# PotatoSpudowski/fastLLaMa

Hardware: NVIDIA H100
Metric: tokens/sec LLaMA-7B q4_0 decode (n_batch=1, greedy) (higher is better)
Workload: dtype u8

## Files before the change

### fastllama_b200/csrc/fl_token_kernel.cu

```cuda
#include <cuda_fp16.h>
#include <stdlib.h>

#include <algorithm>
#include <vector>

#include "fl_common.cuh"
#include "fl_decode.h"
#include "fl_decode_dev.cuh"
#include "fl_exact.cuh"
#include "fl_kernels.h"

#define TK_CW 16
#define TK_NT (TK_CW * 32)
#define TK_TG 4
#define TK_WPG 4
#define TK_GMAX 4
#define TK_CHB 32
#define TK_PW 4
#define TK_THREADS (TK_NT + 32 * TK_PW)
#define TK_REGS_CONSUMER 104
#define TK_REGS_PRODUCER 64

enum { TK_PH_MATVEC = 0, TK_PH_ATTN = 1 };

struct tk_phase {
    int kind;
    int nb, nchunks;
    uint32_t srow;
    int swiglu;
    int units[3];
    uint32_t row_bytes;
    fl_mv_args a;
    const float *q, *kcache, *vcache;
    float *out;
    int k_row_stride, n_head, head_dim, n_ctx;
    int head_split;
    int out_ll, out_seq, n_out_peer;
    float *out_peer[7];
    float scale;
};

struct tk_params {
    const tk_phase *phases;
    int n_phases;
    unsigned *grid_bar;
    unsigned *err;
    int rank, world;
    unsigned *ll_count;
    int n_ll;
    const uint16_t *exp_tab;
    unsigned long long *prof;
    unsigned *prof2;
    int S, Sg;
    uint32_t grid_magic, grid_shift, s_magic, s_shift;
    uint32_t slot_bytes;
    int diag;
    uint32_t off_y, off_red, off_rowbuf, off_cnt, off_sc, off_stage0;
};

__device__ __forceinline__ unsigned long long tk_now() {
    unsigned long long t;
    asm volatile("mov.u64 %0, %globaltimer;" : "=l"(t));
    return t;
}
__device__ __forceinline__ void tk_bar_consumers(int id) { asm volatile("bar.sync %0, %1;" ::"r"(id), "r"(TK_NT) : "memory"); }

__device__ __forceinline__ void tk_wait_ge(const unsigned *p, unsigned target, bool sys, unsigned *err, unsigned who) {
    unsigned long long t0 = 0;
    for (unsigned n = 1;; n++) {
        unsigned v;
        if (sys) asm volatile("ld.relaxed.sys.global.u32 %0, [%1];" : "=r"(v) : "l"(p) : "memory");
        else asm volatile("ld.acquire.gpu.global.u32 %0, [%1];" : "=r"(v) : "l"(p) : "memory");
        if ((int)(v - target) >= 0) return;
        if ((n & 1023u) == 0) {
            if (*(volatile unsigned *)err) return;
            const unsigned long long t = tk_now();
            if (t0 == 0) t0 = t;
            else if (t - t0 > 2000000000ull) {
                if (atomicExch(err, 1u) == 0u) { err[1] = who; err[2] = target; err[3] = v; err[4] = blockIdx.x; }
                return;
            }
        }
    }
}
__device__ __forceinline__ void tk_mbar_wait(uint32_t bar, uint32_t parity, unsigned *err, unsigned who, unsigned slot) {
    unsigned long long t0 = 0;
    for (unsigned n = 1; !fl_mbar_try_wait(bar, parity); n++) {
        if ((n & 4095u) == 0) {
            if (*(volatile unsigned *)err) return;
            const unsigned long long t = tk_now();
            if (t0 == 0) t0 = t;
            else if (t - t0 > 2000000000ull) {
                if (atomicExch(err, 1u) == 0u) { err[1] = who; err[2] = slot; err[3] = parity; err[4] = blockIdx.x; }
                return;
            }
        }
    }
}
__device__ __forceinline__ void tk_tag_wait(volatile uint32_t *tag, uint32_t want, unsigned *err, unsigned who, unsigned slot) {
    unsigned long long t0 = 0;
    for (unsigned n = 1; *tag != want; n++) {
        if ((n & 4095u) == 0) {
            if (*(volatile unsigned *)err) return;
            const unsigned long long t = tk_now();
            if (t0 == 0) t0 = t;
            else if (t - t0 > 2000000000ull) {
                if (atomicExch(err, 1u) == 0u) { err[1] = who; err[2] = slot; err[3] = want; err[4] = blockIdx.x; }
                return;
            }
        }
    }
}
__device__ __forceinline__ void tk_grid_sync(const tk_params &prm, unsigned target, unsigned) {
    tk_bar_consumers(13);
    if (threadIdx.x == 0) {
        asm volatile("red.release.gpu.global.add.u32 [%0], 1;" ::"l"(prm.grid_bar) : "memory");
        tk_wait_ge(prm.grid_bar, target, false, prm.err, 0x100u);
    }
    tk_bar_consumers(13);
}

struct tk_slice {
    int f0, f1, f2, n0, n1, n2, t0, t1, ntiles;
};
__device__ __forceinline__ uint32_t tk_div(uint32_t n, uint32_t magic, uint32_t shift) { return (magic ? __umulhi(n, magic) : n) >> shift; }
__device__ __forceinline__ tk_slice tk_make_slice_u(int m0, int m1, int m2, int lgG, uint32_t grid_magic, uint32_t grid_shift) {
    tk_slice sl;
    const unsigned U = (unsigned)(m0 + m1 + m2);
    const int u0 = (int)tk_div(U * blockIdx.x, grid_magic, grid_shift);
    const int u1 = (int)tk_div(U * (blockIdx.x + 1), grid_magic, grid_shift);
    const int rnd = (1 << lgG) - 1;
    fd_seg_span(u0, u1, 0, m0, sl.f0, sl.n0);
    fd_seg_span(u0, u1, m0, m1, sl.f1, sl.n1);
    fd_seg_span(u0, u1, m0 + m1, m2, sl.f2, sl.n2);
    sl.t0 = (sl.n0 + rnd) >> lgG;
    sl.t1 = sl.t0 + ((sl.n1 + rnd) >> lgG);
    sl.ntiles = sl.t1 + ((sl.n2 + rnd) >> lgG);
    return sl;
}
__device__ __forceinline__ void tk_tile_of(const tk_slice &sl, int G, int t, int &seg, int &unit0, int &nunits) {
    seg = (t < sl.t0) ? 0 : (t < sl.t1) ? 1 : 2;
    const int j = t - (seg == 0 ? 0 : seg == 1 ? sl.t0 : sl.t1);
    const int first = seg == 0 ? sl.f0 : seg == 1 ? sl.f1 : sl.f2;
    const int n = seg == 0 ? sl.n0 : seg == 1 ? sl.n1 : sl.n2;
    unit0 = first + j * G;
    nunits = min(G, n - j * G);
}

typedef fl_yx tk_yblock;

template <int E>
__device__ __forceinline__ void tk_load_vals(const float4 *p4, int u, float v[E], bool cg) {
#pragma unroll
    for (int k = 0; k < E / 4; k++) {
        const float4 t = cg ? __ldcg(p4 + (E / 4) * u + k) : __ldg(p4 + (E / 4) * u + k);
        v[4 * k + 0] = t.x; v[4 * k + 1] = t.y; v[4 * k + 2] = t.z; v[4 * k + 3] = t.w;
    }
}
template <int E>
__device__ __forceinline__ void tk_zero_vals(float v[E]) {
#pragma unroll
    for (int k = 0; k < E; k++) v[k] = 0.f;
}
template <int E>
__device__ __forceinline__ void tk_load_ll(const float *base, int u, float v[E], unsigned e, unsigned *err) {
    const uint4 *p = (const uint4 *)base + (size_t)(E / 2) * u;
    unsigned long long t0 = 0;
    for (unsigned n = 1;; n++) {
        uint4 t[E / 2];
#pragma unroll
        for (int k = 0; k < E / 2; k++)
            asm volatile("ld.relaxed.sys.global.v4.u32 {%0, %1, %2, %3}, [%4];" : "=r"(t[k].x), "=r"(t[k].y), "=r"(t[k].z), "=r"(t[k].w) : "l"(p + k) : "memory");
        bool ok = true;
#pragma unroll
        for (int k = 0; k < E / 2; k++) {
            ok = ok && t[k].y == e && t[k].w == e;
            v[2 * k] = __uint_as_float(t[k].x);
            v[2 * k + 1] = __uint_as_float(t[k].z);
        }
        if (ok) return;
        __nanosleep(n < 4 ? 40u : 200u);
        if ((n & 255u) == 0) {
            if (*(volatile unsigned *)err) return;
            const unsigned long long now = tk_now();
            if (t0 == 0) t0 = now;
            else if (now - t0 > 2000000000ull) {
                if (atomicExch(err, 1u) == 0u) { err[1] = 0x300u; err[2] = e; err[3] = t[0].y; err[4] = blockIdx.x; }
                return;
            }
        }
    }
}
template <int E>
__device__ __forceinline__ void tk_load_x(const fl_mv_args &A, int u, float v[E], unsigned ll_epoch, unsigned *err) {
    if (A.x_ll) tk_load_ll<E>(A.x, u, v, ll_epoch, err);
    else tk_load_vals<E>((const float4 *)A.x, u, v, true);
    if (A.xadd) {
        float w[E];
        tk_load_vals<E>((const float4 *)A.xadd, u, w, true);
#pragma unroll
        for (int k = 0; k < E; k++) v[k] = __fadd_rn(v[k], w[k]);
    }
}
template <int E>
__device__ __forceinline__ void tk_store_vals(float *dst, int u, const float v[E]) {
#pragma unroll
    for (int k = 0; k < E / 4; k++) ((float4 *)dst)[(E / 4) * u + k] = make_float4(v[4 * k], v[4 * k + 1], v[4 * k + 2], v[4 * k + 3]);
}
template <int E>
__device__ __forceinline__ void tk_quant(const float v[E], int u, bool valid, tk_yblock *ysm, int off) {
    float m0 = 0.f, m1 = 0.f;
#pragma unroll
    for (int k = 0; k < E; k += 2) { m0 = fmaxf(m0, fabsf(v[k])); m1 = fmaxf(m1, fabsf(v[k + 1])); }
    float amax = fmaxf(m0, m1);
    if (E <= 16) amax = fmaxf(amax, __shfl_xor_sync(0xffffffffu, amax, 1));
    if (E == 8) amax = fmaxf(amax, __shfl_xor_sync(0xffffffffu, amax, 2));
    const float d = __fdiv_rn(amax, 127.f);
    const float id = (amax != 0.0f) ? __fdiv_rn(127.f, amax) : 0.0f;
    int q[E], s0 = 0, s1 = 0;
#pragma unroll
    for (int k = 0; k < E; k += 2) {
        q[k] = max(-128, min(127, __float2int_rn(__fmul_rn(v[k], id))));
        q[k + 1] = max(-128, min(127, __float2int_rn(__fmul_rn(v[k + 1], id))));
        s0 += q[k]; s1 += q[k + 1];
    }
    int sum = s0 + s1;
    if (E <= 16) sum += __shfl_xor_sync(0xffffffffu, sum, 1);
    if (E == 8) sum += __shfl_xor_sync(0xffffffffu, sum, 2);
    if (valid) {
        constexpr int NW = E / 8;
        constexpr int UPB = 32 / E;
        tk_yblock *yb = ysm + u / UPB;
        const int part = u % UPB;
#pragma unroll
        for (int j = 0; j < NW; j++) {
            const uint32_t ya = (uint32_t)(q[8 * j + 0] & 0xFF) | ((uint32_t)(q[8 * j + 1] & 0xFF) << 8) | ((uint32_t)(q[8 * j + 2] & 0xFF) << 16) | ((uint32_t)(q[8 * j + 3] & 0xFF) << 24);
            const uint32_t yb4 = (uint32_t)(q[8 * j + 4] & 0xFF) | ((uint32_t)(q[8 * j + 5] & 0xFF) << 8) | ((uint32_t)(q[8 * j + 6] & 0xFF) << 16) | ((uint32_t)(q[8 * j + 7] & 0xFF) << 24);
            const int sa = q[8 * j + 0] + q[8 * j + 1] + q[8 * j + 2] + q[8 * j + 3], sb = q[8 * j + 4] + q[8 * j + 5] + q[8 * j + 6] + q[8 * j + 7];
            *(uint4 *)yb->q[NW * part + j] = make_uint4(ya, yb4, (uint32_t)(FX_MAGIC_I - off * sa), (uint32_t)(FX_MAGIC_I - off * sb));
        }
        if (part == 0) *(float2 *)&yb->d = make_float2(d, __fmul_rn(d, (float)sum));
    }
}
template <int E>
__device__ __forceinline__ void tk_prologue_nonorm(const fl_mv_args &A, int K, tk_yblock *ysm, int warp, int tid, unsigned lle, unsigned *err) {
    const int qoff = (A.type == FL_TYPE_Q4_0) ? 8 : 0;
    const int nu = K / E;
    if (E == 16 && A.pro != FL_PRO_SILUMUL && nu > TK_NT && nu <= 2 * TK_NT) {
        const int ua = tid, ub = tid + TK_NT;
        const bool vb = ub < nu, wb = TK_NT + warp * 32 < nu;
        float va[E], vv[E];
        tk_load_x<E>(A, ua, va, lle, err);
        if (vb) tk_load_x<E>(A, ub, vv, lle, err); else tk_zero_vals<E>(vv);
        if (A.sum_out && blockIdx.x == 0) { tk_store_vals<E>(A.sum_out, ua, va); if (vb) tk_store_vals<E>(A.sum_out, ub, vv); }
        tk_quant<E>(va, ua, true, ysm, qoff);
        if (wb) tk_quant<E>(vv, ub, vb, ysm, qoff);
        return;
    }
    for (int u0 = 0; u0 < nu; u0 += TK_NT) {
        if (u0 + warp * 32 >= nu) break;
        const int u = u0 + tid;
        const bool valid = u < nu;
        float v[E];
        if (valid) tk_load_x<E>(A, u, v, lle, err); else tk_zero_vals<E>(v);
        if (A.sum_out && blockIdx.x == 0 && valid) tk_store_vals<E>(A.sum_out, u, v);
        if (A.pro == FL_PRO_SILUMUL) {
            float bm[E];
            if (valid) tk_load_vals<E>((const float4 *)A.b, u, bm, true); else tk_zero_vals<E>(bm);
#pragma unroll
            for (int k = 0; k < E; k++) {
                const uint16_t hh = __half_as_ushort(__float2half_rn(v[k]));
                v[k] = __fmul_rn(__half2float(__ushort_as_half(__ldg(A.silu_tab + hh))), bm[k]);
            }
        }
        tk_quant<E>(v, u, valid, ysm, qoff);
    }
}

template <int RES>
__device__ __forceinline__ void tk_prologue_norm(const fl_mv_args &A, int K, tk_yblock *ysm, double *red, int warp, int lane, int tid, unsigned lle, unsigned *err) {
    const int qoff = (A.type == FL_TYPE_Q4_0) ? 8 : 0;
    constexpr int E = 8, NR = RES > 0 ? RES : 1;
    const int nu = K >> 3;
    float v[NR][E], gm[NR][E];
    double acc = 0.0;
    if (RES > 0) {
#pragma unroll
        for (int r = 0; r < NR; r++) {
            const int u = tid + r * TK_NT;
            if (u < nu) { tk_load_x<E>(A, u, v[r], lle, err); tk_load_vals<E>((const float4 *)A.gamma, u, gm[r], false); }
            else { tk_zero_vals<E>(v[r]); tk_zero_vals<E>(gm[r]); }
        }
#pragma unroll
        for (int r = 0; r < NR; r++)
#pragma unroll
            for (int k = 0; k < E; k++) acc += (double)__fmul_rn(v[r][k], v[r][k]);
    } else {
        for (int u = tid; u < nu; u += TK_NT) {
            tk_load_x<E>(A, u, v[0], lle, err);
#pragma unroll
            for (int k = 0; k < E; k++) acc += (double)__fmul_rn(v[0][k], v[0][k]);
        }
    }
    acc = fl_warp_sum_d(acc);
    if (lane == 0) red[warp] = acc;
    tk_bar_consumers(15);
    if (warp == 0) {
        double t = 0.0;
#pragma unroll
        for (int w = 0; w < TK_CW; w++) t += red[w];
        const float mean = (float)(t / (double)K);
        if (lane == 0) ((float *)(red + 16))[0] = __fdiv_rn(1.0f, __fsqrt_rn(__fadd_rn(mean, 1e-6f)));
    }
    tk_bar_consumers(15);
    const float scale = ((float *)(red + 16))[0];
    if (RES > 0) {
#pragma unroll
        for (int r = 0; r < NR; r++) {
            if (r * TK_NT + warp * 32 < nu) {
                const int u = tid + r * TK_NT;
                const bool valid = u < nu;
                if (A.sum_out && blockIdx.x == 0 && valid) tk_store_vals<E>(A.sum_out, u, v[r]);
#pragma unroll
                for (int k = 0; k < E; k++) v[r][k] = __fmul_rn(gm[r][k], __fmul_rn(v[r][k], scale));
                if (A.normed_out && blockIdx.x == 0 && valid) tk_store_vals<E>(A.normed_out, u, v[r]);
                tk_quant<E>(v[r], u, valid, ysm, qoff);
            }
        }
    } else {
        for (int u0 = 0; u0 < nu; u0 += TK_NT) {
            if (u0 + warp * 32 >= nu) break;
            const int u = u0 + tid;
            const bool valid = u < nu;
            if (valid) { tk_load_x<E>(A, u, v[0], lle, err); tk_load_vals<E>((const float4 *)A.gamma, u, gm[0], false); }
            else { tk_zero_vals<E>(v[0]); tk_zero_vals<E>(gm[0]); }
            if (A.sum_out && blockIdx.x == 0 && valid) tk_store_vals<E>(A.sum_out, u, v[0]);
#pragma unroll
            for (int k = 0; k < E; k++) v[0][k] = __fmul_rn(gm[0][k], __fmul_rn(v[0][k], scale));
            if (A.normed_out && blockIdx.x == 0 && valid) tk_store_vals<E>(A.normed_out, u, v[0]);
            tk_quant<E>(v[0], u, valid, ysm, qoff);
        }
    }
}

__device__ __forceinline__ void tk_prologue(const fl_mv_args &A, int K, tk_yblock *ysm, double *red, int warp, int lane, int tid, unsigned lle, unsigned *err) {
    const int nu8 = K >> 3;
    if (A.pro == FL_PRO_RMSNORM) {
        if (nu8 <= TK_NT) tk_prologue_norm<1>(A, K, ysm, red, warp, lane, tid, lle, err);
        else if (nu8 <= 2 * TK_NT) tk_prologue_norm<2>(A, K, ysm, red, warp, lane, tid, lle, err);
        else tk_prologue_norm<0>(A, K, ysm, red, warp, lane, tid, lle, err);
    } else if (nu8 <= TK_NT) {
        tk_prologue_nonorm<8>(A, K, ysm, warp, tid, lle, err);
    } else {
        tk_prologue_nonorm<16>(A, K, ysm, warp, tid, lle, err);
    }
}

__device__ __forceinline__ void tk_store_ll(float *slot, int row, float v, unsigned e, float *const *peers, int n_peers) {
    const unsigned uv = __float_as_uint(v);
    asm volatile("st.relaxed.sys.global.v2.u32 [%0], {%1, %2};" ::"l"(slot + 2 * row), "r"(uv), "r"(e) : "memory");
    for (int r = 0; r < n_peers; r++)
        asm volatile("st.relaxed.sys.global.v2.u32 [%0], {%1, %2};" ::"l"(peers[r] + 2 * row), "r"(uv), "r"(e) : "memory");
}
__device__ __forceinline__ float2 tk_epilogue_preload(const tk_phase &ph, int seg, int u, int n_past) {
    const fl_mv_args &A = ph.a;
    if (ph.swiglu) return make_float2(0.f, 0.f);
    const int r2 = 2 * u;
    if (A.epi == FL_EPI_QKV) {
        if (seg < 2) return __ldg((const float2 *)A.rope_cs + (size_t)n_past * (A.head_dim >> 1) + ((r2 % A.head_dim) >> 1));
        return make_float2(0.f, 0.f);
    }
    if (A.epi == FL_EPI_RESADD) {
        if (A.res_ll) {
            const float4 t = __ldcg((const float4 *)(A.res + 2 * r2));
            return make_float2(t.x, t.z);
        }
        return __ldcg((const float2 *)(A.res + r2));
    }
    return make_float2(0.f, 0.f);
}
__device__ __forceinline__ void tk_epilogue(const tk_phase &ph, int seg, int u, float a, float b, int n_past, float2 pre, unsigned ll_epoch) {
    const fl_mv_args &A = ph.a;
    if (ph.swiglu) {
        const uint16_t h = __half_as_ushort(__float2half_rn(a));
        const float o = __fmul_rn(__half2float(__ushort_as_half(__ldg(A.silu_tab + h))), b);
        if (A.out_ll) tk_store_ll(A.seg_dst[0], u, o, ll_epoch, A.dst_peer, A.n_dst_peer);
        else A.seg_dst[0][u] = o;
        return;
    }
    const int r2 = 2 * u;
    if (A.epi == FL_EPI_QKV) {
        if (seg < 2) {
            const float2 cs = pre;
            const float y0 = __fmaf_rn(a, cs.x, -__fmul_rn(b, cs.y));
            const float y1 = __fmaf_rn(a, cs.y, __fmul_rn(b, cs.x));
            float *o = (seg == 0) ? (A.seg_dst[0] + r2) : (A.kcache + (size_t)n_past * A.n_embd + r2);
            *(float2 *)o = make_float2(y0, y1);
        } else {
            A.vcache[(size_t)r2 * A.n_ctx + n_past] = a;
            A.vcache[(size_t)(r2 + 1) * A.n_ctx + n_past] = b;
        }
        return;
    }
    if (A.epi == FL_EPI_RESADD) {
        a = __fadd_rn(a, pre.x);
        b = __fadd_rn(b, pre.y);
    }
    if (A.out_ll) {
        tk_store_ll(A.seg_dst[seg], r2, a, ll_epoch, A.dst_peer, A.n_dst_peer);
        tk_store_ll(A.seg_dst[seg], r2 + 1, b, ll_epoch, A.dst_peer, A.n_dst_peer);
        return;
    }
    *(float2 *)(A.seg_dst[seg] + r2) = make_float2(a, b);
}

struct tk_stream {
    int first, n_g;
};
__device__ __forceinline__ tk_stream tk_stream_of(int g, int T0, int ntasks) {
    tk_stream st;
    st.first = ((g - (T0 & 3)) + 4) & 3;
    st.n_g = st.first < ntasks ? (ntasks - st.first + 3) >> 2 : 0;
    return st;
}
__device__ __forceinline__ void tk_slot_of(const tk_params &prm, int g, uint32_t idx, int &s, uint32_t &par) {
    const uint32_t q = tk_div(idx, prm.s_magic, prm.s_shift);
    s = (int)(idx - q * (uint32_t)prm.Sg) * TK_TG + g;
    par = q & 1u;
}

__device__ __forceinline__ unsigned tk_clock() {
    unsigned c;
    asm volatile("mov.u32 %0, %%clock;" : "=r"(c));
    return c;
}
template <int TYPE, bool PROF>
__device__ __forceinline__ void tk_consume(const tk_phase &ph, const tk_params &prm, const tk_slice &sl, int T0, uint32_t &cg, const tk_yblock *ysm,
                                           uint8_t *stage0, volatile uint32_t *tags, uint32_t bar0, int warp, int lane, unsigned *pw, unsigned lle) {
    unsigned c_begin = 0, c_wait = 0, c_dot = 0, c_tail = 0, c_rounds = 0, c_t = 0;
    if (PROF) { c_begin = tk_clock(); c_t = c_begin; }
    constexpr int BB = (TYPE == FL_TYPE_Q4_0) ? 20 : 24, QOFF = (TYPE == FL_TYPE_Q4_0) ? 4 : 8;
    const fl_mv_args &A = ph.a;
    const int S = prm.S;
    const int g = warp % TK_TG, wl = warp / TK_TG;
    const int r = lane >> 2, jj = lane & 3;
    const bool swiglu = ph.swiglu != 0;
    const int C = ph.nchunks, nb = ph.nb;
    const tk_stream st = tk_stream_of(g, T0, sl.ntiles);
    const int n_past = (A.epi == FL_EPI_QKV) ? *A.n_past : 0;
    const bool leader = swiglu ? ((lane & 3) == 0 && lane < 16) : ((lane & 7) == 0);
    const int pr = swiglu ? (lane >> 2) : (lane >> 3);
    const uint32_t row_off = (uint32_t)r * ph.srow + (uint32_t)(QOFF + 4 * jj);
    for (int k = wl; k < st.n_g; k += TK_WPG) {
        const int k0 = k - wl, n_r = min(TK_WPG, st.n_g - k0);
        int seg, unit0, nunits;
        tk_tile_of(sl, TK_GMAX, st.first + 4 * k, seg, unit0, nunits);
        float2 pre = make_float2(0.f, 0.f);
        if (leader && pr < nunits) pre = tk_epilogue_preload(ph, seg, unit0 + pr, n_past);
        float a0 = 0.0f, a1 = 0.0f, sm = 0.0f;
        for (int c = 0; c < C; c++) {
            int s;
            uint32_t par;
            const uint32_t idx = cg + (uint32_t)(k0 * C + c * n_r + wl);
            tk_slot_of(prm, g, idx, s, par);
            tk_tag_wait(tags + s, idx + 1u, prm.err, 0x600u + (unsigned)warp, (unsigned)s);
            tk_mbar_wait(bar0 + 8u * s, par, prm.err, 0x400u + (unsigned)warp, (unsigned)s);
            if (PROF) { const unsigned t = tk_clock(); c_wait += t - c_t; c_t = t; c_rounds++; }
            if (!(prm.diag & 2)) {
                const uint8_t *wp = stage0 + (size_t)s * prm.slot_bytes + row_off;
                const tk_yblock *yp = ysm + c * TK_CHB;
                const int nbc = min(TK_CHB, nb - c * TK_CHB);
#pragma unroll 8
                for (int i = 0; i < nbc; i++) {
                    const uint32_t w = *(const uint32_t *)(wp + i * BB);
                    const float dx = *(const float *)(wp + i * BB - (QOFF + 4 * jj));
                    const uint4 y = *(const uint4 *)yp[i].q[jj];
                    const float2 ds = *(const float2 *)&yp[i].d;
                    if (TYPE == FL_TYPE_Q4_1) sm = __fmaf_rn(*(const float *)(wp + i * BB - (QOFF + 4 * jj) + 4), ds.y, sm);
                    fx_block(w, __fmul_rn(dx, ds.x), y, a0, a1);
                }
            }
            __syncwarp();
            if (lane == 0) fl_mbar_arrive(bar0 + 8u * (S + s));
            if (PROF) { const unsigned t = tk_clock(); c_dot += t - c_t; c_t = t; }
        }
        float tot = fx_reduce(a0, a1);
        if (TYPE == FL_TYPE_Q4_1) tot = __fadd_rn(tot, sm);
        const float other = __shfl_down_sync(0xffffffffu, tot, swiglu ? 16 : 4);
        if (leader && pr < nunits) tk_epilogue(ph, seg, unit0 + pr, tot, other, n_past, pre, lle);
        if (PROF) { const unsigned t = tk_clock(); c_tail += t - c_t; c_t = t; }
    }
    cg += (uint32_t)(st.n_g * C);
    if (PROF && lane == 0 && pw) {
        pw[0] = 0; pw[1] = c_wait; pw[2] = c_dot; pw[3] = c_tail; pw[4] = c_rounds; pw[5] = tk_clock() - c_begin; pw[6] = (unsigned)sl.ntiles; pw[7] = 0;
    }
}

__device__ __forceinline__ void tk_attention(const tk_phase &ph, const tk_params &prm, float *sc, double *red, int head, int part_id, int warp, int lane, int tid, unsigned lle_out) {
    float *redf = (float *)(red + 20);
    const int hd = ph.head_dim;
    const int n_pos = *ph.a.n_past + 1;
    const float *q = ph.q + (size_t)head * hd;
    const float *kbase = ph.kcache + (size_t)head * hd;
    if (hd == 128) {
        float qe[4];
#pragma unroll
        for (int c = 0; c < 4; c++) qe[c] = __ldcg(q + lane + 32 * c);
        for (int j0 = warp * 8; j0 < n_pos; j0 += TK_CW * 8) {
            float kv[8][4], acc[8];
#pragma unroll
            for (int u = 0; u < 8; u++)
#pragma unroll
                for (int c = 0; c < 4; c++) kv[u][c] = __ldcg(kbase + (size_t)min(j0 + u, n_pos - 1) * ph.k_row_stride + lane + 32 * c);
#pragma unroll
            for (int u = 0; u < 8; u++) {
                acc[u] = 0.f;
#pragma unroll
                for (int c = 0; c < 4; c++) acc[u] = __fmaf_rn(kv[u][c], qe[c], acc[u]);
            }
#pragma unroll
            for (int u = 0; u < 8; u++) {
                const float a = fx_reduce_f32(acc[u]);
                if (lane == 0 && j0 + u < n_pos) sc[j0 + u] = __fmul_rn(a, ph.scale);
            }
        }
    } else {
        for (int j0 = warp * 4; j0 < n_pos; j0 += TK_CW * 4) {
            float acc[4] = {0.f, 0.f, 0.f, 0.f};
            for (int e = lane; e < hd; e += 32) {
                const float qe = __ldcg(q + e);
#pragma unroll
                for (int u = 0; u < 4; u++) acc[u] = __fmaf_rn(__ldcg(kbase + (size_t)min(j0 + u, n_pos - 1) * ph.k_row_stride + e), qe, acc[u]);
            }
#pragma unroll
            for (int u = 0; u < 4; u++) {
                const float a = fx_reduce_f32(acc[u]);
                if (lane == 0 && j0 + u < n_pos) sc[j0 + u] = __fmul_rn(a, ph.scale);
            }
        }
    }
    tk_bar_consumers(12);
    float mx = -INFINITY;
    for (int j = tid; j < n_pos; j += TK_NT) mx = fmaxf(mx, sc[j]);
    mx = fl_warp_max(mx);
    if (lane == 0) redf[warp] = mx;
    tk_bar_consumers(12);
    mx = redf[0];
    for (int w = 1; w < TK_CW; w++) mx = fmaxf(mx, redf[w]);
    double sum = 0.0;
    for (int j = tid; j < n_pos; j += TK_NT) {
        const uint16_t hh = __half_as_ushort(__float2half_rn(__fsub_rn(sc[j], mx)));
        const float e = __half2float(__ushort_as_half(__ldg(prm.exp_tab + hh)));
        sc[j] = e;
        sum += (double)e;
    }
    sum = fl_warp_sum_d(sum);
    if (lane == 0) red[warp] = sum;
    tk_bar_consumers(12);
    double tot = 0.0;
    for (int w = 0; w < TK_CW; w++) tot += red[w];
    const float inv = (float)(1.0 / tot);
    for (int j = tid; j < n_pos; j += TK_NT) sc[j] = __fmul_rn(sc[j], inv);
    tk_bar_consumers(12);
    const int dpc = hd / ph.head_split;
    const int np = n_pos & ~31, rem = n_pos - np, nma = fx_left_nma(rem);
    for (int dl = warp; dl < dpc; dl += TK_CW) {
        const int d = part_id * dpc + dl;
        const float *vrow = ph.vcache + ((size_t)head * hd + d) * ph.n_ctx;
        float acc = 0.0f;
        const float lx = (lane < rem) ? __ldcg(vrow + np + lane) : 0.0f, ly = (lane < rem) ? sc[np + lane] : 0.0f;
        const float lv = __fmul_rn(lx, ly);
        for (int k = lane; k < np; k += 32) acc = __fmaf_rn(__ldcg(vrow + k), sc[k], acc);
        float o = fx_reduce_f32(acc);
        for (int k = 0; k < nma; k++) o = __fadd_rn(o, __shfl_sync(0xffffffffu, lv, k));
        for (int k = nma; k < rem; k++) o = __fmaf_rn(__shfl_sync(0xffffffffu, lx, k), __shfl_sync(0xffffffffu, ly, k), o);
        if (lane == 0) {
            if (ph.out_ll) tk_store_ll(ph.out, head * hd + d, o, lle_out, ph.out_peer, ph.n_out_peer);
            else ph.out[(size_t)head * hd + d] = o;
        }
    }
}
__device__ __forceinline__ void tk_attention_prefetch(const tk_phase &ph, int head, int part_id, int tid) {
    const int hd = ph.head_dim, n_past = *ph.a.n_past;
    const int kl = (hd * 4 + 127) / 128;
    for (int i = tid; i < n_past * kl; i += TK_NT) {
        const float *p = ph.kcache + (size_t)(i / kl) * ph.k_row_stride + (size_t)head * hd + (i % kl) * 32;
        asm volatile("prefetch.global.L2 [%0];" ::"l"(p));
    }
    const int dpc = hd / ph.head_split;
    const int vl = (n_past * 4 + 127) / 128;
    for (int i = tid; i < dpc * vl; i += TK_NT) {
        const float *p = ph.vcache + ((size_t)head * hd + part_id * dpc + i / vl) * ph.n_ctx + (i % vl) * 32;
        asm volatile("prefetch.global.L2 [%0];" ::"l"(p));
    }
}

template <bool PROF>
__global__ void __launch_bounds__(TK_THREADS, 1) k_decode_token(const tk_params prm) {
    extern __shared__ __align__(128) uint8_t smem[];
    uint64_t *bars = (uint64_t *)smem;
    volatile uint32_t *tags = (volatile uint32_t *)(smem + (size_t)16 * prm.S);
    tk_yblock *ysm = (tk_yblock *)(smem + prm.off_y);
    double *red = (double *)(smem + prm.off_red);
    float *sc = (float *)(smem + prm.off_sc);
    uint8_t *stage0 = smem + prm.off_stage0;
    __shared__ __align__(16) tk_phase phs[2];
    __shared__ tk_slice sl_sh;
    const int S = prm.S;
    const int warp = threadIdx.x >> 5, lane = threadIdx.x & 31;
    const uint32_t bar0 = fl_smem_u32(bars);

    if (warp >= TK_CW) {
        asm volatile("setmaxnreg.dec.sync.aligned.u32 %0;" ::"n"(TK_REGS_PRODUCER));
        const int pg = warp - TK_CW;
        if (pg == 0 && lane == 0) {
            for (int s = 0; s < S; s++) {
                fl_mbar_init(bar0 + 8u * s, 1);
                fl_mbar_init(bar0 + 8u * (S + s), 1);
                tags[s] = 0u;
            }
            fl_mbar_fence_init();
        }
        __syncwarp();
        asm volatile("bar.sync 14, %0;" ::"r"(TK_THREADS) : "memory");
        {
            const uint64_t pol = fl_policy_evict_first();
            int T0 = 0;
            uint32_t cg = 0;
            for (int pi = 0; pi < prm.n_phases; pi++) {
                const tk_phase *gp = prm.phases + pi;
                if (__ldg(&gp->kind) != TK_PH_MATVEC) continue;
                const int swiglu = __ldg(&gp->swiglu), C = __ldg(&gp->nchunks), nb = __ldg(&gp->nb), type = __ldg(&gp->a.type);
                const int m0 = __ldg(&gp->units[0]), m1 = __ldg(&gp->units[1]), m2 = __ldg(&gp->units[2]);
                const uint32_t row_bytes = __ldg(&gp->row_bytes), srow = __ldg(&gp->srow);
                const uint32_t bb = (type == FL_TYPE_Q4_0) ? 20u : 24u;
                const uint8_t *w0 = (const uint8_t *)__ldg((const unsigned long long *)&gp->a.seg_w[0]);
                const uint8_t *w1 = (const uint8_t *)__ldg((const unsigned long long *)&gp->a.seg_w[1]);
                const uint8_t *w2 = (const uint8_t *)__ldg((const unsigned long long *)&gp->a.seg_w[2]);
                const tk_slice sl = tk_make_slice_u(m0, m1, m2, 2, prm.grid_magic, prm.grid_shift);
                const tk_stream st = tk_stream_of(pg, T0, sl.ntiles);
                for (int k0 = 0; k0 < st.n_g; k0 += TK_WPG) {
                    const int n_r = min(TK_WPG, st.n_g - k0);
                    for (int c = 0; c < C; c++) {
                        const uint32_t cbytes = (uint32_t)min(TK_CHB, nb - c * TK_CHB) * bb;
                        for (int wl = 0; wl < n_r; wl++) {
                            int seg, unit0, nunits;
                            tk_tile_of(sl, TK_GMAX, st.first + 4 * (k0 + wl), seg, unit0, nunits);
                            int s;
                            uint32_t par;
                            const uint32_t idx = cg + (uint32_t)(k0 * C + c * n_r + wl);
                            tk_slot_of(prm, pg, idx, s, par);
                            const uint8_t *src = nullptr;
                            if (lane < 8) {
                                if (swiglu) { if ((lane & 3) < nunits) src = ((lane < 4) ? w0 : w1) + (size_t)(unit0 + (lane & 3)) * row_bytes; }
                                else if (lane < 2 * nunits) src = (seg == 0 ? w0 : seg == 1 ? w1 : w2) + (size_t)(2 * unit0 + lane) * row_bytes;
                            }
                            if (lane == 0) {
                                tk_mbar_wait(bar0 + 8u * (S + s), par ^ 1u, prm.err, 0x500u + (unsigned)pg, (unsigned)s);
                                tags[s] = idx + 1u;
                                if (prm.diag & 1) fl_mbar_arrive(bar0 + 8u * s);
                                else fl_mbar_expect_tx(bar0 + 8u * s, 2u * (uint32_t)nunits * cbytes);
                            }
                            __syncwarp();
                            if (src && !(prm.diag & 1))
                                fl_bulk_g2s_hint(fl_smem_u32(stage0 + (size_t)s * prm.slot_bytes + (size_t)lane * srow), src + (size_t)c * (TK_CHB * bb), cbytes, bar0 + 8u * s, pol);
                        }
                    }
                }
                cg += (uint32_t)(st.n_g * C);
                T0 += sl.ntiles;
            }
        }
        return;
    }

    asm volatile("setmaxnreg.inc.sync.aligned.u32 %0;" ::"n"(TK_REGS_CONSUMER));
    const int tid = threadIdx.x;
    static_assert(sizeof(tk_phase) % 4 == 0 && sizeof(tk_phase) / 4 <= TK_NT, "descriptor copy is one word per thread");
    if (warp == TK_CW - 1)
        for (int i = lane; i < (int)(sizeof(tk_phase) / 4); i += 32) ((uint32_t *)&phs[0])[i] = ((const uint32_t *)&prm.phases[0])[i];
    tk_bar_consumers(15);
    asm volatile("bar.sync 14, %0;" ::"r"(TK_THREADS) : "memory");
    int T0 = 0;
    uint32_t cg = 0;
    unsigned epoch = 0;
    unsigned ll_base = 0;
    if (prm.n_ll > 0) asm volatile("ld.relaxed.gpu.global.u32 %0, [%1];" : "=r"(ll_base) : "l"(prm.ll_count) : "memory");
    unsigned *err = prm.err;
    for (int pi = 0; pi < prm.n_phases; pi++) {
        const tk_phase &ph = phs[pi & 1];
        unsigned long long *pr = (prm.prof && tid == 0) ? prm.prof + ((size_t)pi * gridDim.x + blockIdx.x) * 4 : nullptr;
        if (pr) pr[0] = tk_now();
        const bool attn_here = ph.kind == TK_PH_ATTN && (int)blockIdx.x < ph.n_head * ph.head_split;
        const int a_head = attn_here ? (int)blockIdx.x / ph.head_split : 0, a_part = attn_here ? (int)blockIdx.x % ph.head_split : 0;
        if (attn_here) tk_attention_prefetch(ph, a_head, a_part, tid);
        const bool ll_in = ph.kind == TK_PH_MATVEC && ph.a.x_ll;
        const unsigned lle_in = ll_in ? ll_base + (unsigned)ph.a.x_seq + 1u : 0u;
        const unsigned lle_out = ph.kind == TK_PH_MATVEC ? (ph.a.out_ll ? ll_base + (unsigned)ph.a.out_seq + 1u : 0u) : (ph.out_ll ? ll_base + (unsigned)ph.out_seq + 1u : 0u);
        if (pi > 0 && ll_in) {
            tk_bar_consumers(13);
        } else if (pi > 0) {
            epoch++;
            if (!(prm.diag & 4)) tk_grid_sync(prm, epoch * gridDim.x, 0u);
            else tk_bar_consumers(13);
        }
        if (pr) pr[1] = tk_now();
        uint32_t next_word = 0;
        const bool copies = tid < (int)(sizeof(tk_phase) / 4) && pi + 1 < prm.n_phases;
        if (copies) next_word = __ldcg((const uint32_t *)&prm.phases[pi + 1] + tid);
        if (ph.kind == TK_PH_ATTN) {
            if (attn_here && !(prm.diag & 16)) tk_attention(ph, prm, sc, red, a_head, a_part, warp, lane, tid, lle_out);
            if (copies) ((uint32_t *)&phs[(pi + 1) & 1])[tid] = next_word;
            tk_bar_consumers(15);
            if (pr) pr[2] = pr[3] = tk_now();
            continue;
        }
        const int K = ph.nb * 32;
        if (tid == TK_NT - 1) sl_sh = tk_make_slice_u(ph.units[0], ph.units[1], ph.units[2], 2, prm.grid_magic, prm.grid_shift);
        if (!(prm.diag & 8)) tk_prologue(ph.a, K, ysm, red, warp, lane, tid, lle_in, err);
        if (copies) ((uint32_t *)&phs[(pi + 1) & 1])[tid] = next_word;
        tk_bar_consumers(15);
        if (pr) pr[2] = tk_now();
        const tk_slice &sl = sl_sh;
        unsigned *pw = (PROF && prm.prof2) ? prm.prof2 + (((size_t)pi * gridDim.x + blockIdx.x) * TK_CW + warp) * 8 : nullptr;
        if (ph.a.type == FL_TYPE_Q4_0) tk_consume<FL_TYPE_Q4_0, PROF>(ph, prm, sl, T0, cg, ysm, stage0, tags, bar0, warp, lane, pw, lle_out);
        else                           tk_consume<FL_TYPE_Q4_1, PROF>(ph, prm, sl, T0, cg, ysm, stage0, tags, bar0, warp, lane, pw, lle_out);
        T0 += sl.ntiles;
        if (pr) pr[3] = tk_now();
    }
    if (prm.n_ll > 0 && blockIdx.x == 0 && tid == 0) *prm.ll_count = ll_base + (unsigned)prm.n_ll;
}

struct fl_token_plan_impl {
    tk_phase *d_phases = nullptr;
    unsigned *d_bar = nullptr;
    unsigned *h_err = nullptr;
    unsigned long long *d_prof = nullptr;
    unsigned *d_prof2 = nullptr;
    tk_params prm;
    size_t smem = 0;
    int n_kernels = 0;
};

static void tk_magic(uint32_t d, uint32_t &magic, uint32_t &shift) {
    uint32_t k = 0;
    while ((2u << k) <= d) k++;
    shift = k;
    magic = ((d & (d - 1)) == 0) ? 0u : (uint32_t)((((uint64_t)1 << (32 + k)) + d - 1) / d);
}

static int tk_geometry(tk_phase &ph, size_t &tile_bytes) {
    const fl_mv_args &a = ph.a;
    const int bb = fl_block_bytes(a.type);
    const int nb = a.K / 32;
    const size_t row_bytes = a.row_stride_bytes ? a.row_stride_bytes : (size_t)nb * bb;
    FL_REQUIRE(bb > 0 && a.K > 0 && a.K % 32 == 0 && row_bytes % 16 == 0, "token kernel: unsupported matrix K=%d", a.K);
    const uint32_t chunk_bytes = (uint32_t)std::min(nb, TK_CHB) * bb;
    FL_REQUIRE(chunk_bytes % 16 == 0 && ((size_t)nb * bb) % 16 == 0, "token kernel: K=%d gives row pieces that are not multiples of 16 bytes", a.K);
    const uint32_t srow = (chunk_bytes / 16) % 2 ? chunk_bytes : chunk_bytes + 16;
    ph.units[0] = ph.units[1] = ph.units[2] = 0;
    if (ph.swiglu) {
        ph.units[0] = a.seg_rows[0];
    } else {
        for (int i = 0; i < a.nseg; i++) {
            FL_REQUIRE(a.seg_rows[i] > 0 && a.seg_rows[i] % 2 == 0, "token kernel: segment %d has an odd row count", i);
            ph.units[i] = a.seg_rows[i] / 2;
        }
    }
    for (int i = 0; i < a.nseg; i++) {
        FL_REQUIRE(((uintptr_t)a.seg_w[i] & 15) == 0, "token kernel: segment %d is not 16-byte aligned", i);
        FL_REQUIRE(a.epi == FL_EPI_QKV || ph.swiglu || ((uintptr_t)a.seg_dst[i] & 7) == 0, "token kernel: output %d is not 8-byte aligned", i);
    }
    FL_REQUIRE(a.epi != FL_EPI_RESADD || ((uintptr_t)a.res & 7) == 0, "token kernel: residual is not 8-byte aligned");
    FL_REQUIRE((long)ph.units[0] + ph.units[1] + ph.units[2] < (1 << 23), "token kernel: too many rows");
    ph.kind = TK_PH_MATVEC;
    ph.nb = nb; ph.nchunks = (nb + TK_CHB - 1) / TK_CHB; ph.srow = srow; ph.row_bytes = (uint32_t)row_bytes;
    tile_bytes = (size_t)2 * TK_GMAX * srow;
    return 0;
}

int flk_token_plan_create(const fl_token_step *steps, int n_steps, const uint16_t *silu_tab, const uint16_t *exp_tab, const void *rope_cs, unsigned *epoch_counter, void **out) {
    std::vector<tk_phase> phases((size_t)n_steps);
    for (int i = 0; i < n_steps; i++) {
        tk_phase &ph = phases[i];
        memset(&ph, 0, sizeof(ph));
        if (steps[i].kind == 1) {
            ph.kind = TK_PH_ATTN;
            ph.q = steps[i].q; ph.kcache = steps[i].kcache; ph.vcache = steps[i].vcache; ph.out = steps[i].out;
            ph.k_row_stride = steps[i].k_row_stride; ph.n_head = steps[i].n_head; ph.head_dim = steps[i].head_dim; ph.n_ctx = steps[i].n_ctx;
            ph.scale = steps[i].scale;
            ph.a.n_past = steps[i].n_past;
            ph.out_ll = steps[i].out_ll; ph.out_seq = steps[i].out_seq; ph.n_out_peer = steps[i].n_out_peer;
            for (int r = 0; r < 7; r++) ph.out_peer[r] = steps[i].out_peer[r];
        } else {
            ph.kind = TK_PH_MATVEC;
            ph.a = steps[i].mv;
            ph.a.silu_tab = silu_tab;
            ph.a.rope_cs = rope_cs;
        }
    }
    for (int i = 0; i < n_steps; i++)
        if (phases[i].kind == TK_PH_MATVEC && phases[i].a.swiglu) {
            const fl_mv_args &a = phases[i].a;
            FL_REQUIRE(a.nseg == 2 && a.epi == FL_EPI_STORE && a.seg_rows[0] == a.seg_rows[1], "token kernel: a swiglu step needs two equal segments and a plain store");
            phases[i].swiglu = 1;
        }
    for (int i = 0; i + 1 < n_steps; i++) {
        tk_phase &p0 = phases[i], &p1 = phases[i + 1];
        if (p0.kind != TK_PH_MATVEC || p1.kind != TK_PH_MATVEC || p0.swiglu) continue;
        const fl_mv_args &a = p0.a;
        if (a.nseg == 2 && a.epi == FL_EPI_STORE && a.seg_rows[0] == a.seg_rows[1] && p1.a.pro == FL_PRO_SILUMUL && p1.a.x == a.seg_dst[0] &&
            p1.a.b == a.seg_dst[1] && p1.a.K == a.seg_rows[0] && p1.a.xadd == nullptr) {
            p0.swiglu = 1;
            p1.a.pro = FL_PRO_PLAIN;
            p1.a.b = nullptr;
        }
    }
    size_t max_tile = 0, max_y = 0;
    int max_ctx = 0;
    int sm_count = 0;
    {
        int dev0 = 0;
        FL_CUDA_OK(cudaGetDevice(&dev0));
        FL_CUDA_OK(cudaDeviceGetAttribute(&sm_count, cudaDevAttrMultiProcessorCount, dev0));
    }
    for (int i = 0; i < n_steps; i++) {
        tk_phase &ph = phases[i];
        if (ph.kind == TK_PH_ATTN) {
            FL_REQUIRE(ph.n_ctx % 4 == 0 && ph.head_dim >= 32 && ph.head_dim <= 256 && (ph.head_dim & (ph.head_dim - 1)) == 0 && ph.n_head <= sm_count,
                       "token kernel: unsupported attention shape");
            ph.head_split = 1;
            for (int c = 4; c > 1; c /= 2)
                if (c * ph.n_head <= sm_count && ph.head_dim / c >= 32) { ph.head_split = c; break; }
            max_ctx = std::max(max_ctx, ph.n_ctx);
        } else {
            size_t tb = 0;
            if (tk_geometry(ph, tb)) return -1;
            max_tile = std::max(max_tile, tb);
            max_y = std::max(max_y, (size_t)ph.nb * sizeof(tk_yblock));
        }
    }
    int dev = 0, sm = 0, optin = 0;
    FL_CUDA_OK(cudaGetDevice(&dev));
    FL_CUDA_OK(cudaDeviceGetAttribute(&sm, cudaDevAttrMultiProcessorCount, dev));
    FL_CUDA_OK(cudaDeviceGetAttribute(&optin, cudaDevAttrMaxSharedMemoryPerBlockOptin, dev));
    fl_token_plan_impl *pl = new fl_token_plan_impl();
    struct plan_guard {
        fl_token_plan_impl *p;
        ~plan_guard() { if (p) flk_token_plan_destroy(p); }
    } guard{pl};
    tk_params &p = pl->prm;
    const size_t slot = (max_tile + 127) & ~(size_t)127;
    int S = 64;
    if (getenv("FASTLLAMA_B200_TK_SLOTS")) S = std::max(8, std::min(64, atoi(getenv("FASTLLAMA_B200_TK_SLOTS")) / 4 * 4));
    size_t off = 0;
    for (;; S -= 4) {
        if (S < 8) { fl_set_error("token kernel: tiles of %zu bytes do not fit shared memory", slot); return -1; }
        p.off_y = ((size_t)(2 * S) * 8 + (size_t)S * 4 + 127) & ~(size_t)127;
        p.off_red = (p.off_y + max_y + 127) & ~(size_t)127;
        p.off_sc = (p.off_red + 32 * sizeof(double) + 127) & ~(size_t)127;
        off = (p.off_sc + ((size_t)max_ctx + 32) * sizeof(float) + 127) & ~(size_t)127;
        if (off + (size_t)S * slot <= (size_t)optin - 1024) break;
    }
    p.off_rowbuf = p.off_cnt = 0;
    p.off_stage0 = (uint32_t)off;
    p.S = S;
    p.Sg = S / TK_TG;
    tk_magic((uint32_t)sm, p.grid_magic, p.grid_shift);
    tk_magic((uint32_t)p.Sg, p.s_magic, p.s_shift);
    p.slot_bytes = (uint32_t)slot;
    p.n_phases = n_steps;
    p.exp_tab = exp_tab;
    p.diag = getenv("FASTLLAMA_B200_TK_DIAG") ? atoi(getenv("FASTLLAMA_B200_TK_DIAG")) : 0;
    pl->smem = off + (size_t)S * slot;
    FL_CUDA_OK(cudaMalloc((void **)&pl->d_phases, sizeof(tk_phase) * (size_t)n_steps));
    FL_CUDA_OK(cudaMemcpy(pl->d_phases, phases.data(), sizeof(tk_phase) * (size_t)n_steps, cudaMemcpyHostToDevice));
    FL_CUDA_OK(cudaMalloc((void **)&pl->d_bar, 256));
    p.phases = pl->d_phases;
    p.grid_bar = pl->d_bar;
    FL_CUDA_OK(cudaMemset(pl->d_bar, 0, 256));
    FL_CUDA_OK(cudaHostAlloc((void **)&pl->h_err, 64, cudaHostAllocMapped));
    memset(pl->h_err, 0, 64);
    FL_CUDA_OK(cudaHostGetDevicePointer((void **)&p.err, pl->h_err, 0));
    p.rank = 0; p.world = 1; p.ll_count = epoch_counter; p.n_ll = 0;
    for (int i = 0; i < n_steps; i++) {
        const tk_phase &ph = phases[i];
        if (ph.kind == TK_PH_MATVEC) {
            if (ph.a.out_ll) p.n_ll = std::max(p.n_ll, ph.a.out_seq + 1);
            if (ph.a.x_ll) p.n_ll = std::max(p.n_ll, ph.a.x_seq + 1);
            if (ph.a.out_ll && ph.a.nseg != 1 && !ph.swiglu) { fl_set_error("token kernel: an LL output needs a single segment (or a w1|w3 pair)"); return -1; }
        } else if (ph.out_ll) p.n_ll = std::max(p.n_ll, ph.out_seq + 1);
    }
    if (p.n_ll > 0 && !epoch_counter) { fl_set_error("token kernel: steps use LL vectors but no epoch counter was given (fl_token_plan_create_ll)"); return -1; }
    p.prof = nullptr;
    p.prof2 = nullptr;
    if (getenv("FASTLLAMA_B200_TOKEN_PROF")) {
        FL_CUDA_OK(cudaMalloc((void **)&pl->d_prof, sizeof(unsigned long long) * 4 * (size_t)n_steps * sm));
        FL_CUDA_OK(cudaMemset(pl->d_prof, 0, sizeof(unsigned long long) * 4 * (size_t)n_steps * sm));
        p.prof = pl->d_prof;
        const size_t n2 = (size_t)n_steps * sm * TK_CW * 8;
        FL_CUDA_OK(cudaMalloc((void **)&pl->d_prof2, n2 * sizeof(unsigned)));
        FL_CUDA_OK(cudaMemset(pl->d_prof2, 0, n2 * sizeof(unsigned)));
        p.prof2 = pl->d_prof2;
    }
    cudaFuncAttributes fa;
    FL_CUDA_OK(cudaFuncGetAttributes(&fa, k_decode_token<false>));
    FL_CUDA_OK(cudaFuncSetAttribute(k_decode_token<false>, cudaFuncAttributeMaxDynamicSharedMemorySize, optin - (int)fa.sharedSizeBytes));
    FL_CUDA_OK(cudaFuncGetAttributes(&fa, k_decode_token<true>));
    FL_CUDA_OK(cudaFuncSetAttribute(k_decode_token<true>, cudaFuncAttributeMaxDynamicSharedMemorySize, optin - (int)fa.sharedSizeBytes));
    FL_REQUIRE((size_t)TK_REGS_CONSUMER * TK_NT + (size_t)TK_REGS_PRODUCER * 32 * TK_PW <= (size_t)fa.numRegs * TK_THREADS,
               "token kernel: register re-allocation (%d x %d + %d x %d) exceeds the launch allocation (%d x %d)", TK_REGS_CONSUMER, TK_NT, TK_REGS_PRODUCER,
               32 * TK_PW, fa.numRegs, TK_THREADS);
    int per_sm = 0;
    FL_CUDA_OK(cudaOccupancyMaxActiveBlocksPerMultiprocessor(&per_sm, k_decode_token<false>, TK_THREADS, pl->smem));
    if (per_sm < 1) { const size_t need = pl->smem; fl_set_error("token kernel: one CTA per SM does not fit (smem %zu)", need); return -1; }
    pl->n_kernels = sm;
    guard.p = nullptr;
    *out = pl;
    return 0;
}

int flk_token_plan_launch(cudaStream_t st, void *plan) {
    fl_token_plan_impl *pl = (fl_token_plan_impl *)plan;
    FL_CUDA_OK(cudaMemsetAsync(pl->d_bar, 0, 4, st));
    void *args[] = {(void *)&pl->prm};
    const void *fn = pl->prm.prof2 ? (const void *)k_decode_token<true> : (const void *)k_decode_token<false>;
    FL_CUDA_OK(cudaLaunchCooperativeKernel(fn, dim3(pl->n_kernels), dim3(TK_THREADS), args, pl->smem, st));
    fl_count_launch();
    return 0;
}

int flk_token_plan_profile(void *plan, unsigned long long *out, size_t max_words, int *n_ctas) {
    fl_token_plan_impl *pl = (fl_token_plan_impl *)plan;
    FL_REQUIRE(pl && pl->d_prof, "token plan was created without FASTLLAMA_B200_TOKEN_PROF");
    const size_t words = (size_t)4 * pl->prm.n_phases * pl->n_kernels;
    FL_REQUIRE(max_words >= words, "profile buffer too small (%zu words needed)", words);
    FL_CUDA_OK(cudaMemcpy(out, pl->d_prof, words * sizeof(unsigned long long), cudaMemcpyDeviceToHost));
    *n_ctas = pl->n_kernels;
    return 0;
}

int flk_token_plan_profile2(void *plan, unsigned *out, size_t max_words) {
    fl_token_plan_impl *pl = (fl_token_plan_impl *)plan;
    FL_REQUIRE(pl && pl->d_prof2, "token plan was created without FASTLLAMA_B200_TOKEN_PROF");
    const size_t words = (size_t)pl->prm.n_phases * pl->n_kernels * TK_CW * 8;
    FL_REQUIRE(max_words >= words, "profile buffer too small (%zu words needed)", words);
    FL_CUDA_OK(cudaMemcpy(out, pl->d_prof2, words * sizeof(unsigned), cudaMemcpyDeviceToHost));
    return 0;
}

int flk_token_plan_error(void *plan) {
    fl_token_plan_impl *pl = (fl_token_plan_impl *)plan;
    if (!pl || !pl->h_err) return 0;
    const volatile unsigned *e = pl->h_err;
    if (e[0])
        fl_set_error("token kernel timeout: %s (code 0x%x), waited for / slot %u, last saw / parity %u, CTA %u, rank %d of %d",
                     (e[1] & 0x700u) == 0x600u ? "consumer warp waiting for a slot tag" : (e[1] & 0x700u) == 0x400u ? "consumer warp waiting for a weight tile" : (e[1] & 0x700u) == 0x500u ? "producer waiting for a free ring slot" :
                     (e[1] & 0x300u) == 0x300u ? "LL vector element" : "grid barrier counter", e[1], e[2], e[3], e[4], pl->prm.rank, pl->prm.world);
    return (int)e[0];
}

int flk_token_plan_destroy(void *plan) {
    fl_token_plan_impl *pl = (fl_token_plan_impl *)plan;
    if (!pl) return 0;
    if (pl->d_phases) cudaFree(pl->d_phases);
    if (pl->d_bar) cudaFree(pl->d_bar);
    if (pl->h_err) cudaFreeHost(pl->h_err);
    if (pl->d_prof) cudaFree(pl->d_prof);
    if (pl->d_prof2) cudaFree(pl->d_prof2);
    delete pl;
    return 0;
}
```

Baseline: 413.6.

## Replace grid barrier before attention with per-head completion counters

Before each attention phase that follows a fused QKV matvec, the full grid barrier is replaced by per-head atomic counters. Each CTA adds the number of q/K/V rows it produced to its head's counter, and an attention CTA waits only until its own head's count reaches the target. The attention K/V prefetch is moved earlier, into the preceding matvec phase, and V rows are prefetched into L1 and read through the L1-caching path. This aims to cut grid-wide barrier latency and to overlap attention with stragglers, at the cost of extra atomics, a larger barrier buffer that is reset on every launch, and more ordering logic that must stay correct.

```diff
diff --git a/fastllama_b200/csrc/fl_token_kernel.cu b/fastllama_b200/csrc/fl_token_kernel.cu
--- a/fastllama_b200/csrc/fl_token_kernel.cu
+++ b/fastllama_b200/csrc/fl_token_kernel.cu
@@ -38,7 +38,10 @@
     int out_ll, out_seq, n_out_peer;
     float *out_peer[7];
     float scale;
+    unsigned head_target;
+    unsigned *head_cnt;
 };
+#define TK_HCNT_STRIDE 32
 
 struct tk_params {
     const tk_phase *phases;
@@ -502,6 +505,13 @@
     const int n_pos = *ph.a.n_past + 1;
     const float *q = ph.q + (size_t)head * hd;
     const float *kbase = ph.kcache + (size_t)head * hd;
+    {
+        const int dpc = hd / ph.head_split, vl = min((n_pos + 31) >> 5, 4);
+        for (int i = tid; i < dpc * vl; i += TK_NT) {
+            const float *p = ph.vcache + ((size_t)head * hd + part_id * dpc + i / vl) * ph.n_ctx + (i % vl) * 32;
+            asm volatile("prefetch.global.L1 [%0];" ::"l"(p));
+        }
+    }
     if (hd == 128) {
         float qe[4];
 #pragma unroll
@@ -568,9 +578,9 @@
         const int d = part_id * dpc + dl;
         const float *vrow = ph.vcache + ((size_t)head * hd + d) * ph.n_ctx;
         float acc = 0.0f;
-        const float lx = (lane < rem) ? __ldcg(vrow + np + lane) : 0.0f, ly = (lane < rem) ? sc[np + lane] : 0.0f;
+        const float lx = (lane < rem) ? __ldca(vrow + np + lane) : 0.0f, ly = (lane < rem) ? sc[np + lane] : 0.0f;
         const float lv = __fmul_rn(lx, ly);
-        for (int k = lane; k < np; k += 32) acc = __fmaf_rn(__ldcg(vrow + k), sc[k], acc);
+        for (int k = lane; k < np; k += 32) acc = __fmaf_rn(__ldca(vrow + k), sc[k], acc);
         float o = fx_reduce_f32(acc);
         for (int k = 0; k < nma; k++) o = __fadd_rn(o, __shfl_sync(0xffffffffu, lv, k));
         for (int k = nma; k < rem; k++) o = __fmaf_rn(__shfl_sync(0xffffffffu, lx, k), __shfl_sync(0xffffffffu, ly, k), o);
@@ -693,12 +703,28 @@
         if (pr) pr[0] = tk_now();
         const bool attn_here = ph.kind == TK_PH_ATTN && (int)blockIdx.x < ph.n_head * ph.head_split;
         const int a_head = attn_here ? (int)blockIdx.x / ph.head_split : 0, a_part = attn_here ? (int)blockIdx.x % ph.head_split : 0;
-        if (attn_here) tk_attention_prefetch(ph, a_head, a_part, tid);
+        const bool gated = ph.kind == TK_PH_ATTN && ph.head_cnt != nullptr;
+        if (attn_here && !gated) tk_attention_prefetch(ph, a_head, a_part, tid);
         const bool ll_in = ph.kind == TK_PH_MATVEC && ph.a.x_ll;
         const unsigned lle_in = ll_in ? ll_base + (unsigned)ph.a.x_seq + 1u : 0u;
         const unsigned lle_out = ph.kind == TK_PH_MATVEC ? (ph.a.out_ll ? ll_base + (unsigned)ph.a.out_seq + 1u : 0u) : (ph.out_ll ? ll_base + (unsigned)ph.out_seq + 1u : 0u);
-        if (pi > 0 && ll_in) {
+        if (pi > 0 && (ll_in || gated)) {
             tk_bar_consumers(13);
+            if (gated) {
+                if (tid == 0) {
+                    asm volatile("fence.acq_rel.gpu;" ::: "memory");
+                    const int hp = ph.head_dim >> 1;
+                    const int f[3] = {sl_sh.f0, sl_sh.f1, sl_sh.f2}, n[3] = {sl_sh.n0, sl_sh.n1, sl_sh.n2};
+                    for (int s = 0; s < 3; s++)
+                        for (int u = f[s]; u < f[s] + n[s];) {
+                            const int h = u / hp, e = min(f[s] + n[s], (h + 1) * hp);
+                            asm volatile("red.relaxed.gpu.global.add.u32 [%0], %1;" ::"l"(ph.head_cnt + TK_HCNT_STRIDE * h), "r"(e - u) : "memory");
+                            u = e;
+                        }
+                    if (attn_here) tk_wait_ge(ph.head_cnt + TK_HCNT_STRIDE * a_head, ph.head_target, false, err, 0x800u);
+                }
+                if (attn_here) tk_bar_consumers(13);
+            }
         } else if (pi > 0) {
             epoch++;
             if (!(prm.diag & 4)) tk_grid_sync(prm, epoch * gridDim.x, 0u);
@@ -721,6 +747,11 @@
         if (copies) ((uint32_t *)&phs[(pi + 1) & 1])[tid] = next_word;
         tk_bar_consumers(15);
         if (pr) pr[2] = tk_now();
+        if (pi + 1 < prm.n_phases) {
+            const tk_phase &nx = phs[(pi + 1) & 1];
+            if (nx.kind == TK_PH_ATTN && nx.head_cnt && (int)blockIdx.x < nx.n_head * nx.head_split)
+                tk_attention_prefetch(nx, (int)blockIdx.x / nx.head_split, (int)blockIdx.x % nx.head_split, tid);
+        }
         const tk_slice &sl = sl_sh;
         unsigned *pw = (PROF && prm.prof2) ? prm.prof2 + (((size_t)pi * gridDim.x + blockIdx.x) * TK_CW + warp) * 8 : nullptr;
         if (ph.a.type == FL_TYPE_Q4_0) tk_consume<FL_TYPE_Q4_0, PROF>(ph, prm, sl, T0, cg, ysm, stage0, tags, bar0, warp, lane, pw, lle_out);
@@ -734,6 +765,7 @@
 struct fl_token_plan_impl {
     tk_phase *d_phases = nullptr;
     unsigned *d_bar = nullptr;
+    size_t bar_bytes = 0;
     unsigned *h_err = nullptr;
     unsigned long long *d_prof = nullptr;
     unsigned *d_prof2 = nullptr;
@@ -873,15 +905,6 @@
     p.exp_tab = exp_tab;
     p.diag = getenv("FASTLLAMA_B200_TK_DIAG") ? atoi(getenv("FASTLLAMA_B200_TK_DIAG")) : 0;
     pl->smem = off + (size_t)S * slot;
-    FL_CUDA_OK(cudaMalloc((void **)&pl->d_phases, sizeof(tk_phase) * (size_t)n_steps));
-    FL_CUDA_OK(cudaMemcpy(pl->d_phases, phases.data(), sizeof(tk_phase) * (size_t)n_steps, cudaMemcpyHostToDevice));
-    FL_CUDA_OK(cudaMalloc((void **)&pl->d_bar, 256));
-    p.phases = pl->d_phases;
-    p.grid_bar = pl->d_bar;
-    FL_CUDA_OK(cudaMemset(pl->d_bar, 0, 256));
-    FL_CUDA_OK(cudaHostAlloc((void **)&pl->h_err, 64, cudaHostAllocMapped));
-    memset(pl->h_err, 0, 64);
-    FL_CUDA_OK(cudaHostGetDevicePointer((void **)&p.err, pl->h_err, 0));
     p.rank = 0; p.world = 1; p.ll_count = epoch_counter; p.n_ll = 0;
     for (int i = 0; i < n_steps; i++) {
         const tk_phase &ph = phases[i];
@@ -892,6 +915,36 @@
         } else if (ph.out_ll) p.n_ll = std::max(p.n_ll, ph.out_seq + 1);
     }
     if (p.n_ll > 0 && !epoch_counter) { fl_set_error("token kernel: steps use LL vectors but no epoch counter was given (fl_token_plan_create_ll)"); return -1; }
+    const char *attn_barrier = getenv("FASTLLAMA_B200_TK_ATTN_BARRIER");
+    std::vector<int> gated;
+    if (p.n_ll == 0 && !(attn_barrier && atoi(attn_barrier) != 0)) {
+        for (int i = 1; i < n_steps; i++) {
+            const tk_phase &at = phases[i];
+            const fl_mv_args &a = phases[i - 1].a;
+            const int rows = at.n_head * at.head_dim;
+            if (at.kind != TK_PH_ATTN || phases[i - 1].kind != TK_PH_MATVEC || a.epi != FL_EPI_QKV || a.nseg != 3 || a.seg_rows[0] != rows ||
+                a.seg_rows[1] != rows || a.seg_rows[2] != rows || a.head_dim != at.head_dim || a.seg_dst[0] != at.q || a.kcache != at.kcache ||
+                a.vcache != at.vcache || a.n_embd != at.k_row_stride || a.n_ctx != at.n_ctx || a.n_past != at.a.n_past)
+                continue;
+            if (!gated.empty() && (phases[gated[0]].n_head != at.n_head || phases[gated[0]].head_dim != at.head_dim)) continue;
+            gated.push_back(i);
+        }
+    }
+    pl->bar_bytes = sizeof(unsigned) * TK_HCNT_STRIDE * (1 + (gated.empty() ? 0 : phases[gated[0]].n_head));
+    FL_CUDA_OK(cudaMalloc((void **)&pl->d_bar, pl->bar_bytes));
+    FL_CUDA_OK(cudaMemset(pl->d_bar, 0, pl->bar_bytes));
+    for (size_t k = 0; k < gated.size(); k++) {
+        tk_phase &at = phases[gated[k]];
+        at.head_cnt = pl->d_bar + TK_HCNT_STRIDE;
+        at.head_target = (unsigned)(k + 1) * 3u * (unsigned)at.head_dim / 2u;
+    }
+    FL_CUDA_OK(cudaMalloc((void **)&pl->d_phases, sizeof(tk_phase) * (size_t)n_steps));
+    FL_CUDA_OK(cudaMemcpy(pl->d_phases, phases.data(), sizeof(tk_phase) * (size_t)n_steps, cudaMemcpyHostToDevice));
+    p.phases = pl->d_phases;
+    p.grid_bar = pl->d_bar;
+    FL_CUDA_OK(cudaHostAlloc((void **)&pl->h_err, 64, cudaHostAllocMapped));
+    memset(pl->h_err, 0, 64);
+    FL_CUDA_OK(cudaHostGetDevicePointer((void **)&p.err, pl->h_err, 0));
     p.prof = nullptr;
     p.prof2 = nullptr;
     if (getenv("FASTLLAMA_B200_TOKEN_PROF")) {
@@ -922,7 +975,7 @@
 
 int flk_token_plan_launch(cudaStream_t st, void *plan) {
     fl_token_plan_impl *pl = (fl_token_plan_impl *)plan;
-    FL_CUDA_OK(cudaMemsetAsync(pl->d_bar, 0, 4, st));
+    FL_CUDA_OK(cudaMemsetAsync(pl->d_bar, 0, pl->bar_bytes, st));
     void *args[] = {(void *)&pl->prm};
     const void *fn = pl->prm.prof2 ? (const void *)k_decode_token<true> : (const void *)k_decode_token<false>;
     FL_CUDA_OK(cudaLaunchCooperativeKernel(fn, dim3(pl->n_kernels), dim3(TK_THREADS), args, pl->smem, st));
@@ -955,7 +1008,7 @@
     const volatile unsigned *e = pl->h_err;
     if (e[0])
         fl_set_error("token kernel timeout: %s (code 0x%x), waited for / slot %u, last saw / parity %u, CTA %u, rank %d of %d",
-                     (e[1] & 0x700u) == 0x600u ? "consumer warp waiting for a slot tag" : (e[1] & 0x700u) == 0x400u ? "consumer warp waiting for a weight tile" : (e[1] & 0x700u) == 0x500u ? "producer waiting for a free ring slot" :
+                     e[1] == 0x800u ? "attention waiting for its head's q, K and V rows" : (e[1] & 0x700u) == 0x600u ? "consumer warp waiting for a slot tag" : (e[1] & 0x700u) == 0x400u ? "consumer warp waiting for a weight tile" : (e[1] & 0x700u) == 0x500u ? "producer waiting for a free ring slot" :
                      (e[1] & 0x300u) == 0x300u ? "LL vector element" : "grid barrier counter", e[1], e[2], e[3], e[4], pl->prm.rank, pl->prm.world);
     return (int)e[0];
 }
```

After: 415.3 (median of 6 runs). No clear change (+0.4%).
